# 0xSameer/ast

Hardware: AMD Instinct MI355X
Metric: speech frames/s (train step) (higher is better)
Workload: dtype f32 storage / f32 accumulate; batched GEMMs as bf16x3 splits on the bf16 MFMA pipe (every f32 operand value represented EXACTLY by three bf16 terms, f32 exponent range, six term products, each product exact to 2^-26: >= float32 on any data); the encoder recurrences multiply the same way (resident we

## Files before the change

### ast_amd/csrc/common.h

```cpp
#pragma once
#include <hip/hip_runtime.h>
#include <stdint.h>
#include <stddef.h>
#include <stdio.h>
#include <string.h>
#include "../../include/astk.h"

namespace astk {

void set_error(const char* fmt, ...);

enum ProfCat { PROF_ATTN_FWD = 0, PROF_ATTN_BWD = 1, PROF_GEMM = 2, PROF_CELL = 3, PROF_DEC_FWD = 4, PROF_DEC_BWD = 5, PROF_NCAT = 6 };
bool prof_enabled();
float* prof_tick_buffer(int which);
void prof_start(int cat, hipStream_t s, double work);
void prof_stop(int cat, hipStream_t s);
void prof_add_bytes(int cat, double bytes);
struct ProfScope {
  int cat; hipStream_t s; bool on;
  ProfScope(int c, hipStream_t st, double work = 0.0) : cat(c), s(st), on(prof_enabled()) { if (on) prof_start(cat, s, work); }
  ~ProfScope() { if (on) prof_stop(cat, s); }
};

#define ASTK_CHECK(cond, ...)            \
// ... 28 lines not shown
  } while (0)

#define ASTK_TRY(expr)        \
  do {                        \
    int r_ = (expr);          \
    if (r_ != 0) return r_;   \
  } while (0)

enum PersistBit { PERSIST_ENC_FWD = 1, PERSIST_ENC_BWD = 2, PERSIST_DEC_FWD = 4, PERSIST_DEC_BWD = 8 };
struct AbortCtl {
  unsigned* word;
  unsigned* status;
  unsigned limit;
  unsigned bit;
};
AbortCtl abort_ctl(unsigned* word, unsigned bit);
int device_cu_count();
enum TuneKey {
  TUNE_GEMM_TILE, TUNE_GEMM_T256_ABOVE, TUNE_GEMM_GRID, TUNE_GEMM_HYBRID, TUNE_GEMM_CHUNK, TUNE_GEMM_CHUNK_DIV, TUNE_GEMM_LOG, TUNE_GEMM_TICKET,
  TUNE_GEMM_DETERMINISTIC, TUNE_GEMM_FORWARD_PAIRS,
  TUNE_CONV_DIRECT0, TUNE_CONV_SEQ_FWD, TUNE_CONV_SEQ_BWD, TUNE_CONV_SEQ_STATS_BLOCKS, TUNE_CONV_SEQ_APPLY_BLOCKS,
  TUNE_DEC_PERSIST, TUNE_DEC_B6_SPLIT, TUNE_DEC_B6_FUSED, TUNE_DEC_WIDE,
  TUNE_LSTM_PERSIST, TUNE_LSTM_HOIST, TUNE_LSTM_X3, TUNE_LSTM_X4, TUNE_LSTM_ROWS32, TUNE_LSTM_OVERLAP_CHUNK, TUNE_LSTM_SIDE_FWD, TUNE_LSTM_SIDE_BWD, TUNE_LSTM_DUO_SIDE,
  TUNE_ROW_LONGK, TUNE_PERSIST_SPIN_LIMIT, TUNE_COLREDUCE_BLOCKS,
  TUNE_COUNT
};
double tune(TuneKey k);
inline bool tune_on(TuneKey k) { return tune(k) != 0.0; }
__device__ __forceinline__ bool abort_seen(const AbortCtl& ab) {
  return __hip_atomic_load(ab.word, __ATOMIC_RELAXED, __HIP_MEMORY_SCOPE_AGENT) != 0;
}
__device__ __forceinline__ void abort_raise(const AbortCtl& ab) {
  __hip_atomic_store(ab.word, 1u, __ATOMIC_RELAXED, __HIP_MEMORY_SCOPE_AGENT);
  __hip_atomic_fetch_or(ab.status, ab.bit, __ATOMIC_RELAXED, __HIP_MEMORY_SCOPE_AGENT);
}

constexpr int AMAX_SLOT_WORDS = 16;
constexpr int AMAX_PSLOT_STRIDE = 16;
constexpr int AMAX_PSLOT_WORDS = AMAX_SLOT_WORDS * AMAX_PSLOT_STRIDE;
static inline unsigned long long* amax_pslot_handle(unsigned long long* p) { return p ? (unsigned long long*)((uintptr_t)p | 1u) : nullptr; }
static inline __host__ __device__ unsigned long long* amax_shard(const unsigned long long* handle, int i) {
  unsigned long long* base = (unsigned long long*)((uintptr_t)handle & ~(uintptr_t)1);
  return base + (i & (AMAX_SLOT_WORDS - 1)) * (((uintptr_t)handle & 1u) ? AMAX_PSLOT_STRIDE : 1);
}

typedef float f32x4 __attribute__((ext_vector_type(4)));
// ... 141 lines not shown
  long sA, sB, sC;
  int lowp;
  const unsigned long long* amaxA;
  const unsigned long long* amaxB;
  unsigned spanA, spanB;
  int kt;
  int tiles_mn;
  long iters_total;
  int bm;
  int cs;
  long chunk_iters;
};
static inline GemmArgs gemm_args(int M, int N, int K, MatView A, MatView B, float* C, long ldc,
                                 const float* bias = nullptr, int mode = GEMM_STORE, int ksplit = 1) {
  GemmArgs g;
  memset(&g, 0, sizeof(g));
  g.A = A; g.B = B; g.C = C; g.ldc = ldc; g.bias = bias; g.M = M; g.N = N; g.K = K;
  g.mode = mode; g.ksplit = ksplit; g.batch = 1;
  return g;
}
static inline GemmArgs lowp(GemmArgs g) { g.lowp = 1; return g; }
static inline GemmArgs with_amax_a(GemmArgs g, const unsigned long long* a) { g.amaxA = a; return g; }
static inline GemmArgs with_amax_b(GemmArgs g, const unsigned long long* b) { g.amaxB = b; return g; }
int gemm_launch(int layout, const GemmArgs& g, hipStream_t s);
const unsigned long long* gemm_amax(const float* p, long rows, long ld, int inner, hipStream_t s);
void gemm_amax_reserve(int n, unsigned long long** slots, unsigned* gen, hipStream_t s);
const unsigned long long* gemm_amax_bound(float bound, hipStream_t s);
void gemm_amax_step_boundary(hipStream_t s);
struct AmaxMatrix { const float* p; long rows, ld; int inner; };
void gemm_amax_many(const AmaxMatrix* m, int n, const unsigned long long** out, hipStream_t s);
int low_precision_gemms();
int gemm_precision_mode();
struct PrecScope {
  PrecScope(int precision, int operands);
  ~PrecScope();
  int prev_p, prev_l;
};
struct GemmForwardScope {
  GemmForwardScope();
  ~GemmForwardScope();
  int prev;
};
struct DetScope {
  explicit DetScope(int requested);
  ~DetScope();
  int prev;
};
bool deterministic_mode();
struct GemmWgCap {
  explicit GemmWgCap(int wgs);
  ~GemmWgCap();
  int prev;
};
constexpr int GEMM_GROUP_MAX = 12;
struct GemmGroup {
  int n;
  int unit;
  int dp_waves;
  int dp_kt;
  long rem_start;
  long iters_total;
  long iter_start[GEMM_GROUP_MAX + 1];
  unsigned* tick;
  int tick_base[GEMM_GROUP_MAX];
  GemmArgs g[GEMM_GROUP_MAX];
};
int gemm_launch_group(int layout, const GemmArgs* list, int n, hipStream_t s);

const unsigned* persist_status_word();
int status_snapshot_launch(float* dst, hipStream_t s);

int fill_zero(void* p, size_t bytes, hipStream_t s);
constexpr int FILL_SEG_MAX = 16;
struct FillSegs { int n; void* p[FILL_SEG_MAX]; size_t bytes[FILL_SEG_MAX]; unsigned val[FILL_SEG_MAX]; unsigned own[FILL_SEG_MAX]; const void* src[FILL_SEG_MAX]; };
static inline void fill_seg_add(FillSegs& f, void* p, size_t bytes) {
  if (bytes > 0 && f.n < FILL_SEG_MAX) { f.p[f.n] = p; f.bytes[f.n] = bytes; f.own[f.n] = 0; f.val[f.n] = 0; f.src[f.n] = nullptr; ++f.n; }
}
static inline void fill_seg_add(FillSegs& f, void* p, size_t bytes, unsigned value) {
  if (bytes > 0 && f.n < FILL_SEG_MAX) { f.p[f.n] = p; f.bytes[f.n] = bytes; f.own[f.n] = 1; f.val[f.n] = value; f.src[f.n] = nullptr; ++f.n; }
}
static inline void fill_seg_add_copy(FillSegs& f, void* p, const void* src, size_t bytes) {
  if (bytes > 0 && f.n < FILL_SEG_MAX) { f.p[f.n] = p; f.bytes[f.n] = bytes; f.own[f.n] = 0; f.val[f.n] = 0; f.src[f.n] = src; ++f.n; }
}
int fill_u32_segments(const FillSegs& f, unsigned value, hipStream_t s);
struct CopySegs { int n; void* dst[FILL_SEG_MAX]; const void* src[FILL_SEG_MAX]; size_t bytes[FILL_SEG_MAX]; };
static inline void copy_seg_add(CopySegs& c, void* dst, const void* src, size_t bytes) {
  if (bytes > 0 && c.n < FILL_SEG_MAX) { c.dst[c.n] = dst; c.src[c.n] = src; c.bytes[c.n] = bytes; ++c.n; }
// ... 186 lines not shown
```

### ast_amd/csrc/gemm.hip

```cpp
#include "common.h"
#include <cstdio>
#include <cstdlib>
#include <algorithm>
#include <atomic>
#include <mutex>
#include <vector>
#include <type_traits>

namespace astk {

namespace {

#ifndef ASTK_GEMM_BK
#define ASTK_GEMM_BK 16
#endif
constexpr int BK = ASTK_GEMM_BK;
#ifndef ASTK_GEMM_RING
#define ASTK_GEMM_RING 4
#endif
#ifndef ASTK_GEMM_RING8
#define ASTK_GEMM_RING8 2
#endif
#ifndef ASTK_GEMM_PRIO8
#define ASTK_GEMM_PRIO8 3
// ... 58 lines not shown
}
__device__ __forceinline__ void split2(float x0, float x1, unsigned& hi, unsigned& mid, unsigned& lo) {
  hi = cvt_pk_bf16(x0, x1);
  const float r0 = x0 - __uint_as_float(hi << 16), r1 = x1 - __uint_as_float(hi & 0xffff0000u);
  mid = cvt_pk_bf16(r0, r1);
  const float s0 = r0 - __uint_as_float(mid << 16), s1 = r1 - __uint_as_float(mid & 0xffff0000u);
  lo = cvt_pk_bf16(s0, s1);
}
__device__ __forceinline__ int scale_exp(const unsigned long long* amax) {
  if (amax == nullptr) return 127;
  const int st = ((uintptr_t)amax & 1u) ? AMAX_PSLOT_STRIDE : 1;
  amax = (const unsigned long long*)((uintptr_t)amax & ~(uintptr_t)1);
  unsigned long long w = amax[0];
#pragma unroll
  for (int i = 1; i < 16; ++i) w = max(w, amax[i * st]);
  const int e = (int)(((unsigned)w) >> 23) & 0xff;
  return e == 0 ? 127 : min(max(268 - e, 1), 253);
}
constexpr int sp_hs(int TL) { return TL * 16 + 16; }
constexpr int sp_rs(int TL) { return TL * 2 + 64; }
constexpr int sp_plane(int TL, bool RK) { return RK ? (BK / 8) * sp_hs(TL) : BK * sp_rs(TL); }
constexpr int sp_stage(int TL, bool RK, int prec = PREC_BF16X3) { return prec_planes(prec) * sp_plane(TL, RK); }

template <int TL, bool RK, bool TWOLVL, int PREC = PREC_F32, int RING = 1>
struct Stager {
  static constexpr int LD_KR = ld_kr(TL);
  static constexpr int KQ = BK / 4;
  static constexpr int CQ = TL / 4;
  static constexpr int RP = 256 / CQ;
  static constexpr int NP = RK ? TL * KQ / 256 : BK / RP;
  static_assert(NP >= 1 && (RK || RP * NP == BK), "tile / thread-count mismatch");
  float4 reg[RING][NP];
  unsigned voff[NP];
  int tgrp, trem;
  int tcol;
  int a, b;
  int kcur;
  int lds;
  float scl;

  __device__ __forceinline__ void init(const MatView& v, int row0, int nrows, int kbeg, int kend, int tid) {
    kcur = kbeg;
    if (RK) {
      a = tid % KQ;
      b = tid / KQ;
#pragma unroll
      for (int p = 0; p < NP; ++p) voff[p] = (unsigned)((rowoff(v, min(row0 + NP * b + p, nrows - 1)) + a * 4) * 4);
      lds = NP * b * LD_RK + 2 * a;
    } else {
      a = tid % CQ;
      b = tid / CQ;
      const int m = (TL == 128 && PREC == PREC_F32) ? ((a >> 3) & 1) * 64 + (a >> 4) * 32 + (a & 7) * 4 : 4 * a;
      const int col = min(row0 + m, ((nrows + 3) & ~3) - 4);
#pragma unroll
      for (int p = 0; p < NP; ++p)
        voff[p] = (unsigned)(((long)(b + RP * p) * (TWOLVL ? v.st : v.ld) + col) * 4);
      if (TWOLVL) { tgrp = kbeg / v.tn; trem = kbeg % v.tn; tcol = col; }
      lds = b * LD_KR + 4 * a;
    }
  }
  __device__ __forceinline__ void load(const MatView& v, unsigned span, int kend, const int slot = 0) {
    if (RK || !TWOLVL) {
      const long adv = RK ? (long)kcur : (long)kcur * v.ld;
      const __amdgpu_buffer_rsrc_t r =
          __builtin_amdgcn_make_buffer_rsrc(const_cast<float*>(v.p + adv), 0, (int)(span - (unsigned)(adv * 4)), 0x00020000);
#pragma unroll
      for (int p = 0; p < NP; ++p) {
        const u32x4 u = __builtin_amdgcn_raw_buffer_load_b128(r, (int)voff[p], 0, 0);
        reg[slot][p] = make_float4(__uint_as_float(u.x), __uint_as_float(u.y), __uint_as_float(u.z), __uint_as_float(u.w));
      }
    } else {
      if (trem + BK <= v.tn && kcur + BK <= kend) {
        const __amdgpu_buffer_rsrc_t r =
            __builtin_amdgcn_make_buffer_rsrc(const_cast<float*>(v.p + (long)tgrp * v.sg + (long)trem * v.st), 0, 0x7fffffff, 0x00020000);
#pragma unroll
        for (int p = 0; p < NP; ++p) {
          const u32x4 u = __builtin_amdgcn_raw_buffer_load_b128(r, (int)voff[p], 0, 0);
          reg[slot][p] = make_float4(__uint_as_float(u.x), __uint_as_float(u.y), __uint_as_float(u.z), __uint_as_float(u.w));
        }
      } else {
#pragma unroll
        for (int p = 0; p < NP; ++p) {
          const int kr = min(kcur + b + RP * p, kend - 1);
          reg[slot][p] = *reinterpret_cast<const float4*>(v.p + (long)(kr / v.tn) * v.sg + (long)(kr % v.tn) * v.st + tcol);
        }
      }
      trem += BK;
      while (trem >= v.tn) { trem -= v.tn; ++tgrp; }
    }
    kcur += BK;
  }
  __device__ __forceinline__ void load_pair(const MatView& v, unsigned span, const int slot, bool second) {
    static_assert(RING == 1 || (RING % 2) == 0, "pairs of slots");
    const long adv = (long)kcur;
    const __amdgpu_buffer_rsrc_t r =
        __builtin_amdgcn_make_buffer_rsrc(const_cast<float*>(v.p + adv), 0, (int)(span - (unsigned)(adv * 4)), 0x00020000);
#pragma unroll
    for (int p = 0; p < NP; ++p) {
      const u32x4 u = __builtin_amdgcn_raw_buffer_load_b128(r, (int)voff[p], 0, 0);
      reg[slot][p] = make_float4(__uint_as_float(u.x), __uint_as_float(u.y), __uint_as_float(u.z), __uint_as_float(u.w));
      if (second) {
        const u32x4 w = __builtin_amdgcn_raw_buffer_load_b128(r, (int)voff[p] + BK * 4, 0, 0);
        reg[(slot + 1) % RING][p] = make_float4(__uint_as_float(w.x), __uint_as_float(w.y), __uint_as_float(w.z), __uint_as_float(w.w));
      }
    }
    kcur += 2 * BK;
  }
  __device__ __forceinline__ void store(float* S) const {
    if (RK) {
#pragma unroll
      for (int p = 0; p < NP; ++p) {
        *reinterpret_cast<float2*>(&S[lds + p * LD_RK]) = make_float2(reg[0][p].x, reg[0][p].y);
        *reinterpret_cast<float2*>(&S[lds + p * LD_RK + BK / 2]) = make_float2(reg[0][p].z, reg[0][p].w);
      }
    } else {
#pragma unroll
      for (int p = 0; p < NP; ++p) *reinterpret_cast<float4*>(&S[lds + RP * p * LD_KR]) = reg[0][p];
    }
  }
// ... 48 lines not shown
        if (nv < 3) q[BK / 2] = 0.f;
        if (nv < 4) q[BK / 2 + 1] = 0.f;
      }
    } else if (TWOLVL) {
#pragma unroll
      for (int p = 0; p < NP; ++p)
        if (ktile + b + RP * p >= kend) *reinterpret_cast<float4*>(&S[lds + RP * p * LD_KR]) = make_float4(0.f, 0.f, 0.f, 0.f);
    }
  }
};

#ifndef ASTK_GEMM_TICKET
#ifdef ASTK_TEST_HOOKS
#define ASTK_GEMM_TICKET 1
#else
#define ASTK_GEMM_TICKET 0
#endif
#endif
constexpr int TICK_WAVES = 8;
constexpr unsigned TICK_DONE = 1u << 15;
constexpr int gemm_mw(int TLM) { return TLM == 256 ? 8 : 4; }
constexpr int gemm_threads(int PREC, int TLM = 128) { return PREC != PREC_F32 ? 256 + 64 * gemm_mw(TLM) : 256; }
constexpr int gemm_min_waves(int TL, int PREC, int TLM) { return (PREC != PREC_F32 && TLM == 256) ? 3 : waves_per_simd(TL, PREC); }
template <int TL, bool A_RK, bool B_RK, bool TWOLVL, int PREC, int TLM = TL, bool FIX = false>
__global__ __launch_bounds__(gemm_threads(PREC, TLM), gemm_min_waves(TL, PREC, TLM)) void gemm_f32_kernel(GemmGroup grp) {
  static_assert(!FIX || (PREC == PREC_BF16X3 && TL == 128 && TLM == 128), "the deterministic fix-up is instantiated for the 128 x 128 bf16x3 kernel");
  constexpr int LD_KR = ld_kr(TL);
  constexpr int LDA = A_RK ? LD_RK : LD_KR;
  constexpr int LDB = B_RK ? LD_RK : LD_KR;
  constexpr bool SPLIT = PREC != PREC_F32;
  constexpr int MW = SPLIT ? gemm_mw(TLM) : 4;
  constexpr int WT = TL / 2, WTM = TLM / (MW / 2);
  constexpr int NA = WT / 32;
  constexpr int NAM = WTM / 32;
  constexpr int NPL = prec_planes(PREC);
  static_assert(SPLIT || TLM == TL, "the f32 path runs square tiles");
  constexpr int A_FLOATS = SPLIT ? sp_stage(TLM, A_RK, PREC) / 4 : (A_RK ? TL * LD_RK : BK * LD_KR);
  constexpr int B_FLOATS = SPLIT ? sp_stage(TL, B_RK, PREC) / 4 : (B_RK ? TL * LD_RK : BK * LD_KR);
  constexpr int NST = SPLIT ? 3 : 2;
  __shared__ __attribute__((aligned(16))) float As[NST][A_FLOATS];
  __shared__ __attribute__((aligned(16))) float Bs[NST][B_FLOATS];
  static_assert(BK == 16 || BK == 32, "BK / 2 floats per lane and operand, read as BK / 8 float4");

  const bool producer = SPLIT && threadIdx.x >= 64 * MW;
  const int tid = producer ? threadIdx.x - 64 * MW : threadIdx.x;
  const bool stages = !SPLIT || producer, multiplies = !SPLIT || !producer;
  const int lane = tid & 63, wave = tid >> 6;
// ... 32 lines not shown
      tile = r / g.cs;
      const int kk = (int)(r - tile * g.cs);
      k0 = (int)c * g.cs + kk;
      k1 = (int)min((long)(k0 - kk + g.cs), (long)k0 + (lend - lit));
    } else {
      tile = lit / kt_tile;
      k0 = (int)(lit - tile * kt_tile);
      k1 = (int)min((long)kt_tile, (long)k0 + (lend - lit));
    }
    it += k1 - k0;
    int zb, m0, n0;
    decode_tile(g, tile, TLM, TL, zb, m0, n0);
    const int m0_t = m0, n0_t = n0;
    const int kbeg = k0 * BK;
    const int kend = min(g.K, k1 * BK);
    const bool whole = (k0 == 0) && (k1 == kt_tile);

    MatView A = g.A, B = g.B;
    A.p += (long)zb * g.sA;
    B.p += (long)zb * g.sB;
    float* C = g.C + (long)zb * g.sC;

    constexpr int RING = SPLIT ? (MW == 8 ? ASTK_GEMM_RING8 : ASTK_GEMM_RING) : 1;
    Stager<TLM, A_RK, TWOLVL, PREC, RING> sa;
    Stager<TL, B_RK, TWOLVL, PREC, RING> sb;
    sa.init(A, m0, g.M, kbeg, kend, tid & 255);
    sb.init(B, n0, g.N, kbeg, kend, tid & 255);
    int seA = 127, seB = 127;
    if constexpr (PREC == PREC_F16X2 || PREC == PREC_F16) {
      seA = scale_exp(g.amaxA);
      seB = scale_exp(g.amaxB);
      sa.scl = __uint_as_float((unsigned)seA << 23);
      sb.scl = __uint_as_float((unsigned)seB << 23);
    }

    const int nk = k1 - k0;
    const bool add_bias = g.bias != nullptr && k0 == 0;
    const int mode = !whole || g.mode == GEMM_ACCUM ? GEMM_ATOMIC : g.mode;
    const int tick_idx = (ASTK_GEMM_TICKET && !whole && g.mode == GEMM_STORE && grp.tick != nullptr) ? (grp.tick_base[prob] + (int)tile) * TICK_WAVES : -1;
    const float* const e_bias = add_bias ? g.bias : nullptr;
    const long fix_gs0 = (FIX && !whole) ? grp.iter_start[prob] + tile * kt_tile : -1;
    const int g_mode = g.mode, e_kt = g.kt;
    const int e_M = g.M, e_N = g.N, e_ctn = g.c_tn;
    const long e_ldc = g.ldc, e_csg = g.c_sg, e_cst = g.c_st;
    auto epilogue = [&](f32x16 (&acc)[NAM][NA]) {
      int m0 = m0_t, n0 = n0_t;
      asm volatile("" : "+v"(m0), "+v"(n0));
      if (e_bias) {
#pragma unroll
        for (int j = 0; j < NA; ++j) {
// ... 699 lines not shown
    if (inner <= 0 || nrows <= 0 || J.n >= AMAX_REGIONS) return;
    AmaxRegion& R = J.r[J.n];
    R.p = p; R.nb = nb; R.sb = sb; R.rows = nrows; R.ld = ld; R.inner = inner; R.slot = slot;
    const double bytes = 4.0 * nb * nrows * inner;
    const int blocks = (int)std::min(1024.0, std::max(1.0, bytes / (32.0 * 1024.0)));
    J.blk_start[J.n + 1] = J.blk_start[J.n] + blocks;
    ++J.n;
  };
  const long outer = kr ? K : rows;
  const int inner = kr ? rows : K;
  if (v.tn > 0 || v.rowidx) {
    const long n = span_floats;
    push(v.p, batch, sbatch, n / 1024, 1024, 1024);
    push(v.p + (n / 1024) * 1024, batch, sbatch, 1, 0, (int)(n % 1024));
  } else if (v.ld == inner && batch == 1) {
    const long n = outer * (long)inner;
    push(v.p, 1, 0, n / 1024, 1024, 1024);
    push(v.p + (n / 1024) * 1024, 1, 0, 1, 0, (int)(n % 1024));
  } else {
    push(v.p, batch, sbatch, outer, v.ld, inner);
  }
}

int gemm_launch_group(int layout, const GemmArgs* list, int n, hipStream_t s) {
  ASTK_CHECK(layout == GEMM_NT || layout == GEMM_NN || layout == GEMM_TN, "gemm: bad layout %d", layout);
  ASTK_CHECK(n >= 0 && n <= GEMM_GROUP_MAX, "gemm: group of %d products (max %d)", n, GEMM_GROUP_MAX);
  GemmGroup grp;
  bool twolvl = false, any_store = false;
  long tiles = 0;
  double flops = 0;
  int min_kt = 0x7fffffff;
  const int force_tl = (int)tune(TUNE_GEMM_TILE);
  int prec = default_prec();
  if (low_precision_gemms() != 0 && n > 0) {
    bool all = true;
    for (int i = 0; i < n; ++i) all = all && list[i].lowp != 0;
    if (all) prec = PREC_F16;
  }
  if (prec == PREC_F16X2 && tl_wg_cap > 0) prec = PREC_BF16X3;
  const bool det = tl_det != 0;
  if (det && prec == PREC_F16X2) prec = PREC_BF16X3;
  int TL = 128, TLM = 128;
  for (int pass = 0; pass < 3; ++pass) {
    memset(&grp, 0, sizeof(grp));
    twolvl = any_store = false;
    tiles = 0; flops = 0; min_kt = 0x7fffffff;
    bool tall_ok = true;
    for (int i = 0; i < n; ++i) {
      const GemmArgs& g = list[i];
      if (g.M <= 0 || g.N <= 0 || g.K <= 0 || g.batch <= 0) continue;
      GemmArgs& a = grp.g[grp.n];
      bool tl = false;
      ASTK_TRY(gemm_prepare(layout, g, a, tl, TLM, TL));
      twolvl = twolvl || tl;
      grp.iter_start[grp.n] = grp.iters_total;
      grp.iters_total += a.iters_total;
      tiles += (long)a.tiles_mn * g.batch;
      flops += 2.0 * g.M * g.N * (double)g.K * g.batch;
      any_store = any_store || g.mode == GEMM_STORE;
      min_kt = std::min(min_kt, a.kt);
      tall_ok = tall_ok && cdiv(g.M, 256) * 256 * 10 <= cdiv(g.M, 128) * 128 * 11;
      ++grp.n;
    }
    if (pass > 0) break;
    int max_kt = 0;
    for (int i = 0; i < grp.n; ++i) max_kt = std::max(max_kt, grp.g[i].kt);
    bool small = grp.iters_total < 256L * wgs_per_cu(128) * 10 * (32 / BK) && (tiles < 192 || max_kt <= 12 * (16 / BK > 0 ? 16 / BK : 1));
    if (tl_wg_cap > 0) small = small && 2 * tiles < tl_wg_cap;
    const double big_flops = tune(TUNE_GEMM_T256_ABOVE);
    const bool big = prec == PREC_BF16X3 && BK == 16 && tall_ok && flops >= big_flops && !small;
    int want = force_tl == 64 || force_tl == 128 || force_tl == 256 ? force_tl : (small ? 64 : (big ? 256 : 128));
    if (det && prec == PREC_BF16X3) want = 128;
    if (want == 256 && (prec != PREC_BF16X3 || BK != 16)) want = 128;
    if (want == 64 && prec == PREC_F16) want = 128;
    if (want == 128) break;
    TLM = want;
    TL = want == 256 ? 128 : want;
  }
  if (prec == PREC_F16X2 && flops < g_small_flops.load()) {
    bool given = true;
    for (int i = 0; i < grp.n; ++i) given = given && grp.g[i].amaxA && grp.g[i].amaxB;
    if (!given) prec = PREC_BF16X3;
  }
  const int WGS_PER_CU = wgs_per_cu(TL, prec);
  if (grp.n == 0) return 0;
  for (int i = grp.n; i <= GEMM_GROUP_MAX; ++i) grp.iter_start[i] = grp.iters_total;
  grp.unit = prec != PREC_F32 ? 2 : 1;
  for (int i = 0; i < grp.n; ++i)
    if (grp.g[i].kt & 1) grp.unit = 1;
  if (twolvl) {
    const bool a_kr = layout == GEMM_TN, b_kr = layout != GEMM_NT;
    for (int i = 0; i < grp.n; ++i) {
      GemmArgs& a = grp.g[i];
      if (a_kr && a.A.tn <= 0) { a.A.tn = 0x7fffffff; a.A.sg = 0; a.A.st = a.A.ld; }
      if (b_kr && a.B.tn <= 0) { a.B.tn = 0x7fffffff; a.B.sg = 0; a.B.st = a.B.ld; }
    }
  }
  const int force_g = (int)tune(TUNE_GEMM_GRID);
  const bool forward_rule = tl_forward != 0 || tune(TUNE_GEMM_FORWARD_PAIRS) >= 2;
  long G = tiles;
  bool aligned = true;
  if (grp.iters_total >= 256L * WGS_PER_CU * 10 * (32 / BK)) { G = 256 * WGS_PER_CU; aligned = false; }
  else if (tiles < 160) {
    const long g2 = std::min(256L, grp.iters_total / (4 * (32 / BK)));
    if (g2 > tiles) { G = g2; aligned = false; }
  }
  if (force_g > 0) { G = std::min<long>(force_g, grp.iters_total); aligned = false; }
  if (tl_wg_cap > 0 && G > tl_wg_cap) { G = tl_wg_cap; aligned = false; }
  if (det && prec != PREC_BF16X3) { G = tiles; aligned = true; }
  if (det && !aligned && G > FIX_WGS) G = FIX_WGS;
  if (aligned && grp.n > 1) {
    bool uniform = true;
// ... 22 lines not shown
    }
  }
  if (forward_rule && !aligned && grp.dp_waves == 0 && tune_on(TUNE_GEMM_FORWARD_PAIRS)) {
    int max_kt = 0;
    bool uniform = true;
    for (int i = 0; i < grp.n; ++i) { max_kt = std::max(max_kt, grp.g[i].kt); uniform = uniform && grp.g[i].kt == grp.g[0].kt; }
    const long gmax = std::max(1L, grp.iters_total / std::max(1, max_kt));
    if (G > gmax) G = (uniform && max_kt % (2 * grp.unit) == 0 && G >= 2 * tiles) ? 2 * tiles : gmax;
  }
  const bool chunk_on = tune_on(TUNE_GEMM_CHUNK);
  const int chunk_div = (int)tune(TUNE_GEMM_CHUNK_DIV);
  for (int i = 0; i < grp.n; ++i) { grp.g[i].cs = 0; grp.g[i].chunk_iters = 0; }
  if (chunk_on && !det && grp.n == 1 && !aligned && grp.dp_waves == 0 && grp.g[0].mode != GEMM_STORE && prec != PREC_F32 && tiles * chunk_div <= G && grp.g[0].kt >= 128) {
    GemmArgs& a = grp.g[0];
    const long share = grp.iters_total / G;
    int best = 0;
    for (int c = 2; c <= a.kt; c += 2)
      if (a.kt % c == 0 && c >= share / 2 && c <= share * 2 && (best == 0 || labs(c - share) < labs(best - share))) best = c;
    if (best > 0 && best < a.kt) { a.cs = best; a.chunk_iters = tiles * (long)best; }
  }
  const bool log_shapes = tune_on(TUNE_GEMM_LOG);
  if (log_shapes)
    for (int i = 0; i < grp.n; ++i)
      fprintf(stderr, "astk_gemm layout=%d M=%d N=%d K=%d batch=%d mode=%d twolvl=%d group=%d/%d G=%ld kt=%d tile=%d dp_waves=%d bm=%d cs=%d\n", layout, grp.g[i].M,
              grp.g[i].N, grp.g[i].K, grp.g[i].batch, grp.g[i].mode, (int)twolvl, i, grp.n, G, grp.g[i].kt, TLM * 1000 + TL, grp.dp_waves, grp.g[i].bm, grp.g[i].cs);
  ProfScope prof(PROF_GEMM, s, flops);
  if (prof_enabled()) {
    double bytes = 0;
    for (int i = 0; i < grp.n; ++i) {
      const GemmArgs& a = grp.g[i];
      bytes += 4.0 * a.batch * ((double)a.M * a.K + (double)a.N * a.K + (double)a.M * a.N * (a.mode == GEMM_STORE ? 1 : 2));
    }
    prof_add_bytes(PROF_GEMM, bytes);
  }
  dim3 grid((unsigned)G, 1, 1);
  const bool ticket_on = ASTK_GEMM_TICKET && tune_on(TUNE_GEMM_TICKET);
  grp.tick = nullptr;
  const bool fixup = det && !aligned && prec == PREC_BF16X3 && TL == 128 && TLM == 128;
  bool need_zero = !aligned && any_store && G > 1 && !fixup;
  if (need_zero && ticket_on) {
    long ntiles = 0;
    bool fits = true;
    for (int i = 0; i < grp.n; ++i) {
      grp.tick_base[i] = (int)ntiles;
      ntiles += (grp.iter_start[i + 1] - grp.iter_start[i]) / grp.g[i].kt;
      fits = fits && grp.g[i].kt < (int)TICK_DONE;
    }
    if (fits && ntiles < (1L << 27)) {
// ... 35 lines not shown
    if (log_shapes)
      for (int i = 0; i < J.n; ++i)
        fprintf(stderr, "astk_gemm absmax region %d/%d: %ld x %ld rows (ld %ld) x %d floats = %.1f MB, %d blocks\n", i, J.n, J.r[i].nb, J.r[i].rows, J.r[i].ld,
                J.r[i].inner, 4e-6 * J.r[i].nb * J.r[i].rows * J.r[i].inner, J.blk_start[i + 1] - J.blk_start[i]);
    amax_blocks = J.n > 0 ? J.blk_start[J.n] : 0;
    if (amax_blocks > 0) {
      if (need_zero) hipLaunchKernelGGL(k_absmax_zero, dim3((unsigned)(amax_blocks + (G - 1) * ZERO_PARTS)), dim3(256), 0, s, J, grp, (int)G, TLM, TL, zero_vec ? 1 : 0);
      else hipLaunchKernelGGL(k_absmax, dim3((unsigned)amax_blocks), dim3(256), 0, s, J);
    }
  }
  if (need_zero && amax_blocks == 0) hipLaunchKernelGGL(k_zero_split_tiles, dim3((unsigned)((G - 1) * ZERO_PARTS)), dim3(256), 0, s, grp, (int)G, TLM, TL, zero_vec ? 1 : 0);
#define ASTK_GEMM_LAUNCH(T_, P_, M_)                                                                                              \
  switch (layout) {                                                                                                               \
    case GEMM_NT: hipLaunchKernelGGL((gemm_f32_kernel<T_, true, true, false, P_, M_>), grid, dim3(gemm_threads(P_, M_)), 0, s, grp); break;  \
    case GEMM_NN:                                                                                                                 \
      if (twolvl) hipLaunchKernelGGL((gemm_f32_kernel<T_, true, false, true, P_, M_>), grid, dim3(gemm_threads(P_, M_)), 0, s, grp);  \
      else hipLaunchKernelGGL((gemm_f32_kernel<T_, true, false, false, P_, M_>), grid, dim3(gemm_threads(P_, M_)), 0, s, grp);        \
      break;                                                                                                                      \
    default:                                                                                                                      \
      if (twolvl) hipLaunchKernelGGL((gemm_f32_kernel<T_, false, false, true, P_, M_>), grid, dim3(gemm_threads(P_, M_)), 0, s, grp); \
      else hipLaunchKernelGGL((gemm_f32_kernel<T_, false, false, false, P_, M_>), grid, dim3(gemm_threads(P_, M_)), 0, s, grp);       \
      break;                                                                                                                      \
  }
  if (prec == PREC_F32) {
    if (TL == 64) { ASTK_GEMM_LAUNCH(64, PREC_F32, 64) } else { ASTK_GEMM_LAUNCH(128, PREC_F32, 128) }
  } else if (prec == PREC_F16) { ASTK_GEMM_LAUNCH(128, PREC_F16, 128)
  } else if (prec == PREC_F16X2) {
    if (TL == 64) { ASTK_GEMM_LAUNCH(64, PREC_F16X2, 64) } else { ASTK_GEMM_LAUNCH(128, PREC_F16X2, 128) }
  } else if (TLM == 256) {
    if constexpr (BK == 16) { ASTK_GEMM_LAUNCH(128, PREC_BF16X3, 256) }
  } else if (TL == 64) { ASTK_GEMM_LAUNCH(64, PREC_BF16X3, 64)
  } else if (fixup) {
    switch (layout) {
      case GEMM_NT: hipLaunchKernelGGL((gemm_f32_kernel<128, true, true, false, PREC_BF16X3, 128, true>), grid, dim3(gemm_threads(PREC_BF16X3, 128)), 0, s, grp); break;
      case GEMM_NN:
        if (twolvl) hipLaunchKernelGGL((gemm_f32_kernel<128, true, false, true, PREC_BF16X3, 128, true>), grid, dim3(gemm_threads(PREC_BF16X3, 128)), 0, s, grp);
        else hipLaunchKernelGGL((gemm_f32_kernel<128, true, false, false, PREC_BF16X3, 128, true>), grid, dim3(gemm_threads(PREC_BF16X3, 128)), 0, s, grp);
        break;
      default:
        if (twolvl) hipLaunchKernelGGL((gemm_f32_kernel<128, false, false, true, PREC_BF16X3, 128, true>), grid, dim3(gemm_threads(PREC_BF16X3, 128)), 0, s, grp);
        else hipLaunchKernelGGL((gemm_f32_kernel<128, false, false, false, PREC_BF16X3, 128, true>), grid, dim3(gemm_threads(PREC_BF16X3, 128)), 0, s, grp);
        break;
    }
  } else { ASTK_GEMM_LAUNCH(128, PREC_BF16X3, 128) }
#undef ASTK_GEMM_LAUNCH
  ASTK_LAUNCH_CHECK();
  return 0;
}

int gemm_launch(int layout, const GemmArgs& g, hipStream_t s) { return gemm_launch_group(layout, &g, 1, s); }

void gemm_amax_many(const AmaxMatrix* m, int n, const unsigned long long** out, hipStream_t s) {
  for (int i = 0; i < n; ++i) out[i] = nullptr;
  unsigned long long* ring = amax_ring();
  if (default_prec() != PREC_F16X2 || !ring) return;
  ProfScope prof(PROF_GEMM, s, 0.0);
  AmaxJobs J;
  memset(&J, 0, sizeof(J));
  J.gen = next_amax_gen(s);
  for (int i = 0; i < n; ++i) {
    if (!m[i].p || m[i].rows <= 0 || m[i].inner <= 0) continue;
    if (J.n + 2 > AMAX_REGIONS) {
      hipLaunchKernelGGL(k_absmax, dim3((unsigned)J.blk_start[J.n]), dim3(256), 0, s, J);
      const unsigned gen = J.gen;
      memset(&J, 0, sizeof(J));
      J.gen = gen;
    }
    unsigned long long* slot = ring + AMAX_SLOTS / 2 + (size_t)(g_amax_handle.fetch_add(1) % (AMAX_RING_SLOTS / 2)) * AMAX_SLOT_WORDS;
    amax_add(J, mat(m[i].p, m[i].ld), false, (int)m[i].rows, m[i].inner, 1, 0, 0, slot);
    out[i] = slot;
  }
  if (J.n > 0) hipLaunchKernelGGL(k_absmax, dim3((unsigned)J.blk_start[J.n]), dim3(256), 0, s, J);
}
// ... 82 lines not shown
```

### ast_amd/csrc/lstm.hip

```cpp
#include "common.h"
#include <algorithm>
#include <vector>

namespace astk {

struct PersistCellHost {
  const float *Wl, *Wu, *bias, *zx, *xin, *mask, *WlT, *d_enc, *d_hT, *d_cT;
  float *gates, *C, *HR, *HD, *enc;
  const float* WuT;
  float *PR, *PD;
  const float* PD_up;
  int up_external;
  int reverse_pos, layer;
  unsigned long long* amax;
  float* db;
  long dy_sb, dy_st;
  const unsigned* zx_flags; int zx_s0, zx_cs;
  unsigned* prog; int prog_cs;
  float* db_part;
};
bool lstm_persist_hoisted(int h);
bool lstm_persist_applicable(int T, int B, int h, int nl, int nd);
int lstm_persist_rows(int B, int h, int nl, int nd, bool side);
int lstm_persist_layers_per_launch(int B, int h, int nl, int nd, int rows);
// ... 507 lines not shown
      const int rows_d = lstm_persist_hoisted(h) ? 16 : rows_b;
      j.nby = rows_d == 16 ? (B + 15) / 16 : rows_d == 33 ? 2 * ((B + 31) / 32) : (B + 31) / 32;
      for (int i = 0; i < j.n; ++i) { j.db[i] = cells[i].db; j.part[i] = cells[i].db_part; }
      hipLaunchKernelGGL(k_fold_db, dim3(cdiv(4 * h, 256), j.n), dim3(256), 0, s, j);
      ASTK_LAUNCH_CHECK();
    }
  }
  GemmArgs wg[GEMM_GROUP_MAX];
  int nwg = 0;
  const unsigned long long* ax = (d->x_amax && (((uintptr_t)d->x_amax) & 1u)) ? P.ax : (const unsigned long long*)d->x_amax;
  const unsigned long long* aw0[2] = {nullptr, nullptr};
  {
    AmaxMatrix am[3] = {{ax ? nullptr : x, (long)T * B, (long)P.in, P.in}, {dx ? prm[0].Wu : nullptr, 4L * h, (long)P.in, P.in},
                        {dx && P.nd > 1 ? prm[P.nl].Wu : nullptr, 4L * h, (long)P.in, P.in}};
    const unsigned long long* out[3];
    gemm_amax_many(am, 3, out, s);
    if (!ax) ax = out[0];
    aw0[0] = out[1]; aw0[1] = out[2];
  }
  const unsigned long long* ahb = d->out_bound > 0.f ? gemm_amax_bound(exp2f(ceilf(log2f(d->out_bound))), s) : nullptr;
  const unsigned long long* adz_all[16] = {nullptr};
  if (persist)
    for (int i = 0; i < P.nd * P.nl; ++i) adz_all[i] = dz_amax[i];
  ColsumBatch cb;
  for (int l = P.nl - 1; l >= 0; --l) {
    const bool top = l == P.nl - 1;
    const int in = l == 0 ? P.in : h;
    for (int dd = 0; dd < P.nd && !persist; ++dd)
      ASTK_TRY(transpose_f32(P.WlT[dd][l], 4 * h, prm[dd * P.nl + l].Wl, h, 4 * h, h, s));
    for (int i = T - 1; i >= 0 && !persist; --i) {
      LstmCellBwdArgs cells[2];
      for (int dd = 0; dd < P.nd; ++dd) {
        LstmCellBwdArgs& c = cells[dd];
        memset(&c, 0, sizeof(c));
        c.npairs = 1;
        const bool last = i == T - 1;
        c.p[0].A = last ? nullptr : P.ZG[dd][l] + (size_t)(i + 1) * B * 4 * h;
        c.p[0].lda = 4 * h;
        c.p[0].W = P.WlT[dd][l];
        c.p[0].ldw = 4 * h;
        c.p[0].K = last ? 0 : 4 * h;
        c.B = B; c.h = h;
        c.dh_add = (last && d_hT) ? d_hT + ((size_t)dd * P.nl + l) * bh : nullptr;
        if (top) {
          const int pos = dd == 0 ? i : T - 1 - i;
          c.dy2 = d_enc + (size_t)pos * H + (size_t)dd * h;
// ... 23 lines not shown
        wg[nwg++] = with_amax_b(with_amax_a(gemm_args(4 * h, h, rows - B, mat(dz + (size_t)B * 4 * h, 4 * h), mat(P.HR[dd][l], h), g.dWl, h, nullptr, GEMM_ATOMIC, 1), adz), ahb);
      }
      {
        MatView Xv;
        const float* dzu = dz;
        if (l == 0) {
          Xv = mat(x, in);
          if (dd == 1) {
            hipLaunchKernelGGL(k_gather_rows, dim3(2048), dim3(256), 0, s, P.GATH, dz, rows_inv, rows, h);
            ASTK_LAUNCH_CHECK();
            dzu = P.GATH;
          }
        } else Xv = mat(masks ? P.HD[dd][l - 1] : P.HR[dd][l - 1], h);
        if (l == 0 && (dd == 1 || low_precision_gemms())) {
          ASTK_TRY(gemm_launch(GEMM_TN, with_amax_b(with_amax_a(lowp(gemm_args(4 * h, in, rows, mat(dzu, 4 * h), Xv, g.dWu, in, nullptr, GEMM_ATOMIC, 1)), adz), l == 0 ? ax : nullptr), s));
        } else {
          if (nwg == GEMM_GROUP_MAX) { ASTK_TRY(gemm_launch_group(GEMM_TN, wg, nwg, s)); nwg = 0; }
          wg[nwg++] = with_amax_b(with_amax_a(gemm_args(4 * h, in, rows, mat(dzu, 4 * h), Xv, g.dWu, in, nullptr, GEMM_ATOMIC, 1), adz), l == 0 ? ax : ahb);
        }
      }
      if (!persist) ASTK_TRY(cb.add(g.db, dz, 4 * h, rows, 4 * h, s));
      if (l > 0) {
        if (!persist) ASTK_TRY(gemm_launch(GEMM_NN, with_amax_a(gemm_args(rows, h, 4 * h, mat(dz, 4 * h), mat(p.Wu, h), P.DX[dd], h), adz), s));
      } else if (dx && bside.n == 0) {
        MatView A = dd == 0 ? mat(dz, 4 * h) : mat_idx(dz, 4 * h, rows_inv);
        ASTK_TRY(gemm_launch(GEMM_NN, with_amax_b(with_amax_a(lowp(gemm_args(rows, in, 4 * h, A, mat(p.Wu, in), dx, in, nullptr, dd == 0 ? GEMM_STORE : GEMM_ACCUM)), adz), aw0[dd]), s));
      } else if (dx) {
        if (dd == 0) ASTK_TRY(stream_order((hipStream_t)d->side_stream, s));
        const int i1 = T - bside.n * bside.cs;
        if (i1 > 0) ASTK_TRY(dx_steps(dd, 0, i1, s, adz, aw0[dd]));
      }
    }
  }
  ASTK_TRY(cb.flush(s));
  if (nwg > 0) ASTK_TRY(gemm_launch_group(GEMM_TN, wg, nwg, s));
  if (bside.n > 0) ASTK_TRY(stream_order((hipStream_t)d->side_stream, s));
  return 0;
}

}
```

### ast_amd/csrc/util.hip

```cpp
#include "common.h"
#include <algorithm>
#include <stdarg.h>
#include <vector>
#include <atomic>
#include <mutex>

namespace astk {

static thread_local char g_err[512] = "";

void set_error(const char* fmt, ...) {
  va_list ap;
  va_start(ap, fmt);
  vsnprintf(g_err, sizeof(g_err), fmt, ap);
  va_end(ap);
}
const char* last_error() { return g_err; }

struct ProfState {
  bool on = false;
  std::vector<hipEvent_t> ev[PROF_NCAT];
  double work[PROF_NCAT] = {0, 0, 0, 0, 0, 0};
  double bytes[PROF_NCAT] = {0, 0, 0, 0, 0, 0};
};
// ... 50 lines not shown
    {TUNE_GEMM_CHUNK_DIV, "gemm.chunk_div", 4},
    {TUNE_GEMM_LOG, "gemm.log", 0},
    {TUNE_GEMM_TICKET, "gemm.ticket", 1},
    {TUNE_GEMM_DETERMINISTIC, "gemm.deterministic", 0},
    {TUNE_GEMM_FORWARD_PAIRS, "gemm.forward_pairs", 1},
    {TUNE_CONV_DIRECT0, "conv.direct0", 1},
    {TUNE_CONV_SEQ_FWD, "conv.seq_fwd", 1},
    {TUNE_CONV_SEQ_BWD, "conv.seq_bwd", 1},
    {TUNE_CONV_SEQ_STATS_BLOCKS, "conv.seq_stats_blocks", 1024},
    {TUNE_CONV_SEQ_APPLY_BLOCKS, "conv.seq_apply_blocks", 1024},
    {TUNE_DEC_PERSIST, "dec.persist", 1},
    {TUNE_DEC_B6_SPLIT, "dec.b6_split", 1},
    {TUNE_DEC_B6_FUSED, "dec.b6_fused", 1},
    {TUNE_DEC_WIDE, "dec.wide", 1},
    {TUNE_LSTM_PERSIST, "lstm.persist", 1},
    {TUNE_LSTM_HOIST, "lstm.hoist", 1},
    {TUNE_LSTM_X3, "lstm.x3", 1},
    {TUNE_LSTM_X4, "lstm.x4", 1},
    {TUNE_LSTM_ROWS32, "lstm.rows32", -1},
    {TUNE_LSTM_OVERLAP_CHUNK, "lstm.overlap_chunk", 0},
    {TUNE_LSTM_SIDE_FWD, "lstm.side_fwd", 1},
    {TUNE_LSTM_SIDE_BWD, "lstm.side_bwd", 0},
    {TUNE_LSTM_DUO_SIDE, "lstm.duo_side", 0},
    {TUNE_ROW_LONGK, "row.longk", 2048},
    {TUNE_PERSIST_SPIN_LIMIT, "persist.spin_limit", 0},
    {TUNE_COLREDUCE_BLOCKS, "colreduce.blocks", 256},
};
constexpr bool tune_table_in_order() {
  for (int i = 0; i < TUNE_COUNT; ++i)
    if (g_tune_table[i].key != i) return false;
  return true;
}
static_assert(tune_table_in_order(), "g_tune_table rows must follow enum TuneKey");
static std::atomic<double> g_tune[TUNE_COUNT];
static std::atomic<int> g_tune_init{0};
static void tune_init() {
  if (g_tune_init.load(std::memory_order_acquire)) return;
  static std::mutex mu;
  std::lock_guard<std::mutex> lock(mu);
  if (g_tune_init.load()) return;
  for (int i = 0; i < TUNE_COUNT; ++i) g_tune[i].store(g_tune_table[i].def);
  g_tune_init.store(1, std::memory_order_release);
}
double tune(TuneKey k) { tune_init(); return g_tune[k].load(std::memory_order_relaxed); }
static int tune_find(const char* key) {
  if (!key) return -1;
// ... 752 lines not shown
```

Before: 4.724 million.

## Merge both LSTM direction input-gradient GEMMs into one K-split GEMM

For the bottom bidirectional LSTM layer, the forward and backward input-gradient GEMMs (STORE then ACCUM into dx) are replaced by a single NN GEMM of doubled K. The kernel switches its A/B source pointers at k = 4h, with the backward direction's rows gathered through the inverse row index. This removes one launch and one read-modify-write pass over dx, and gives each tile a longer K loop. The cost is a new kernel instantiation with extra per-load branching and stricter layout and precision preconditions.

```diff
diff --git a/ast_amd/csrc/common.h b/ast_amd/csrc/common.h
--- a/ast_amd/csrc/common.h
+++ b/ast_amd/csrc/common.h
@@ -74,6 +74,7 @@
   TUNE_CONV_DIRECT0, TUNE_CONV_SEQ_FWD, TUNE_CONV_SEQ_BWD, TUNE_CONV_SEQ_STATS_BLOCKS, TUNE_CONV_SEQ_APPLY_BLOCKS,
   TUNE_DEC_PERSIST, TUNE_DEC_B6_SPLIT, TUNE_DEC_B6_FUSED, TUNE_DEC_WIDE,
   TUNE_LSTM_PERSIST, TUNE_LSTM_HOIST, TUNE_LSTM_X3, TUNE_LSTM_X4, TUNE_LSTM_ROWS32, TUNE_LSTM_OVERLAP_CHUNK, TUNE_LSTM_SIDE_FWD, TUNE_LSTM_SIDE_BWD, TUNE_LSTM_DUO_SIDE,
+  TUNE_LSTM_MERGED_DX,
   TUNE_ROW_LONGK, TUNE_PERSIST_SPIN_LIMIT, TUNE_COLREDUCE_BLOCKS,
   TUNE_COUNT
 };
@@ -261,7 +262,11 @@
 static inline GemmArgs lowp(GemmArgs g) { g.lowp = 1; return g; }
 static inline GemmArgs with_amax_a(GemmArgs g, const unsigned long long* a) { g.amaxA = a; return g; }
 static inline GemmArgs with_amax_b(GemmArgs g, const unsigned long long* b) { g.amaxB = b; return g; }
-int gemm_launch(int layout, const GemmArgs& g, hipStream_t s);
+struct GemmKSplit {
+  int k2;
+  MatView A2, B2;
+};
+int gemm_launch(int layout, const GemmArgs& g, hipStream_t s, const GemmKSplit* ks = nullptr);
 const unsigned long long* gemm_amax(const float* p, long rows, long ld, int inner, hipStream_t s);
 void gemm_amax_reserve(int n, unsigned long long** slots, unsigned* gen, hipStream_t s);
 const unsigned long long* gemm_amax_bound(float bound, hipStream_t s);
@@ -302,6 +307,10 @@
   long iter_start[GEMM_GROUP_MAX + 1];
   unsigned* tick;
   int tick_base[GEMM_GROUP_MAX];
+  int k2;
+  MatView A2;
+  const float* B2_p;
+  unsigned spanA2, spanB2;
   GemmArgs g[GEMM_GROUP_MAX];
 };
 int gemm_launch_group(int layout, const GemmArgs* list, int n, hipStream_t s);
diff --git a/ast_amd/csrc/gemm.hip b/ast_amd/csrc/gemm.hip
--- a/ast_amd/csrc/gemm.hip
+++ b/ast_amd/csrc/gemm.hip
@@ -104,7 +104,7 @@
 constexpr int sp_plane(int TL, bool RK) { return RK ? (BK / 8) * sp_hs(TL) : BK * sp_rs(TL); }
 constexpr int sp_stage(int TL, bool RK, int prec = PREC_BF16X3) { return prec_planes(prec) * sp_plane(TL, RK); }
 
-template <int TL, bool RK, bool TWOLVL, int PREC = PREC_F32, int RING = 1>
+template <int TL, bool RK, bool TWOLVL, int PREC = PREC_F32, int RING = 1, bool KS = false>
 struct Stager {
   static constexpr int LD_KR = ld_kr(TL);
   static constexpr int KQ = BK / 4;
@@ -114,6 +114,10 @@
   static_assert(NP >= 1 && (RK || RP * NP == BK), "tile / thread-count mismatch");
   float4 reg[RING][NP];
   unsigned voff[NP];
+  unsigned voff2[KS && RK ? NP : 1];
+  int k2;
+  const float* p2;
+  unsigned span2;
   int tgrp, trem;
   int tcol;
   int a, b;
@@ -121,13 +125,25 @@
   int lds;
   float scl;
 
-  __device__ __forceinline__ void init(const MatView& v, int row0, int nrows, int kbeg, int kend, int tid) {
+  __device__ __forceinline__ void init(const MatView& v, int row0, int nrows, int kbeg, int kend, int tid, int ks = 0, const MatView* v2 = nullptr,
+                                       unsigned sp2 = 0) {
     kcur = kbeg;
+    if constexpr (KS) { k2 = ks; p2 = v2->p; span2 = sp2; }
     if (RK) {
       a = tid % KQ;
       b = tid / KQ;
-#pragma unroll
-      for (int p = 0; p < NP; ++p) voff[p] = (unsigned)((rowoff(v, min(row0 + NP * b + p, nrows - 1)) + a * 4) * 4);
+      if constexpr (KS) {
+        const bool second = kbeg >= k2;
+#pragma unroll
+        for (int p = 0; p < NP; ++p) {
+          const int r = min(row0 + NP * b + p, nrows - 1);
+          voff[p] = (unsigned)(((second ? rowoff(*v2, r) : rowoff(v, r)) + a * 4) * 4);
+          if (k2 < kend) voff2[p] = (unsigned)((rowoff(*v2, r) + a * 4) * 4);
+        }
+      } else {
+#pragma unroll
+        for (int p = 0; p < NP; ++p) voff[p] = (unsigned)((rowoff(v, min(row0 + NP * b + p, nrows - 1)) + a * 4) * 4);
+      }
       lds = NP * b * LD_RK + 2 * a;
     } else {
       a = tid % CQ;
@@ -143,9 +159,12 @@
   }
   __device__ __forceinline__ void load(const MatView& v, unsigned span, int kend, const int slot = 0) {
     if (RK || !TWOLVL) {
-      const long adv = RK ? (long)kcur : (long)kcur * v.ld;
+      cross_k2();
+      const bool src2 = KS && kcur >= k2;
+      const long kk = src2 ? kcur - k2 : kcur;
+      const long adv = RK ? kk : kk * v.ld;
       const __amdgpu_buffer_rsrc_t r =
-          __builtin_amdgcn_make_buffer_rsrc(const_cast<float*>(v.p + adv), 0, (int)(span - (unsigned)(adv * 4)), 0x00020000);
+          __builtin_amdgcn_make_buffer_rsrc(const_cast<float*>((src2 ? p2 : v.p) + adv), 0, (int)((src2 ? span2 : span) - (unsigned)(adv * 4)), 0x00020000);
 #pragma unroll
       for (int p = 0; p < NP; ++p) {
         const u32x4 u = __builtin_amdgcn_raw_buffer_load_b128(r, (int)voff[p], 0, 0);
@@ -172,11 +191,19 @@
     }
     kcur += BK;
   }
+  __device__ __forceinline__ void cross_k2() {
+    if (KS && RK && kcur == k2) {
+#pragma unroll
+      for (int p = 0; p < NP; ++p) voff[p] = voff2[p];
+    }
+  }
   __device__ __forceinline__ void load_pair(const MatView& v, unsigned span, const int slot, bool second) {
     static_assert(RING == 1 || (RING % 2) == 0, "pairs of slots");
-    const long adv = (long)kcur;
+    cross_k2();
+    const bool src2 = KS && kcur >= k2;
+    const long adv = src2 ? (long)(kcur - k2) : (long)kcur;
     const __amdgpu_buffer_rsrc_t r =
-        __builtin_amdgcn_make_buffer_rsrc(const_cast<float*>(v.p + adv), 0, (int)(span - (unsigned)(adv * 4)), 0x00020000);
+        __builtin_amdgcn_make_buffer_rsrc(const_cast<float*>((src2 ? p2 : v.p) + adv), 0, (int)((src2 ? span2 : span) - (unsigned)(adv * 4)), 0x00020000);
 #pragma unroll
     for (int p = 0; p < NP; ++p) {
       const u32x4 u = __builtin_amdgcn_raw_buffer_load_b128(r, (int)voff[p], 0, 0);
@@ -271,7 +298,7 @@
 constexpr int gemm_mw(int TLM) { return TLM == 256 ? 8 : 4; }
 constexpr int gemm_threads(int PREC, int TLM = 128) { return PREC != PREC_F32 ? 256 + 64 * gemm_mw(TLM) : 256; }
 constexpr int gemm_min_waves(int TL, int PREC, int TLM) { return (PREC != PREC_F32 && TLM == 256) ? 3 : waves_per_simd(TL, PREC); }
-template <int TL, bool A_RK, bool B_RK, bool TWOLVL, int PREC, int TLM = TL, bool FIX = false>
+template <int TL, bool A_RK, bool B_RK, bool TWOLVL, int PREC, int TLM = TL, bool FIX = false, bool KS = false>
 __global__ __launch_bounds__(gemm_threads(PREC, TLM), gemm_min_waves(TL, PREC, TLM)) void gemm_f32_kernel(GemmGroup grp) {
   static_assert(!FIX || (PREC == PREC_BF16X3 && TL == 128 && TLM == 128), "the deterministic fix-up is instantiated for the 128 x 128 bf16x3 kernel");
   constexpr int LD_KR = ld_kr(TL);
@@ -350,10 +377,17 @@
     float* C = g.C + (long)zb * g.sC;
 
     constexpr int RING = SPLIT ? (MW == 8 ? ASTK_GEMM_RING8 : ASTK_GEMM_RING) : 1;
-    Stager<TLM, A_RK, TWOLVL, PREC, RING> sa;
-    Stager<TL, B_RK, TWOLVL, PREC, RING> sb;
-    sa.init(A, m0, g.M, kbeg, kend, tid & 255);
-    sb.init(B, n0, g.N, kbeg, kend, tid & 255);
+    Stager<TLM, A_RK, TWOLVL, PREC, RING, KS> sa;
+    Stager<TL, B_RK, TWOLVL, PREC, RING, KS> sb;
+    if constexpr (KS) {
+      MatView B2 = B;
+      B2.p = grp.B2_p;
+      sa.init(A, m0, g.M, kbeg, kend, tid & 255, grp.k2, &grp.A2, grp.spanA2);
+      sb.init(B, n0, g.N, kbeg, kend, tid & 255, grp.k2, &B2, grp.spanB2);
+    } else {
+      sa.init(A, m0, g.M, kbeg, kend, tid & 255);
+      sb.init(B, n0, g.N, kbeg, kend, tid & 255);
+    }
     int seA = 127, seB = 127;
     if constexpr (PREC == PREC_F16X2 || PREC == PREC_F16) {
       seA = scale_exp(g.amaxA);
@@ -1099,7 +1133,7 @@
   }
 }
 
-int gemm_launch_group(int layout, const GemmArgs* list, int n, hipStream_t s) {
+static int gemm_launch_impl(int layout, const GemmArgs* list, int n, hipStream_t s, const GemmKSplit* ks) {
   ASTK_CHECK(layout == GEMM_NT || layout == GEMM_NN || layout == GEMM_TN, "gemm: bad layout %d", layout);
   ASTK_CHECK(n >= 0 && n <= GEMM_GROUP_MAX, "gemm: group of %d products (max %d)", n, GEMM_GROUP_MAX);
   GemmGroup grp;
@@ -1117,6 +1151,7 @@
   if (prec == PREC_F16X2 && tl_wg_cap > 0) prec = PREC_BF16X3;
   const bool det = tl_det != 0;
   if (det && prec == PREC_F16X2) prec = PREC_BF16X3;
+  const bool ks_on = ks && ks->k2 > 0;
   int TL = 128, TLM = 128;
   for (int pass = 0; pass < 3; ++pass) {
     memset(&grp, 0, sizeof(grp));
@@ -1150,6 +1185,7 @@
     if (det && prec == PREC_BF16X3) want = 128;
     if (want == 256 && (prec != PREC_BF16X3 || BK != 16)) want = 128;
     if (want == 64 && prec == PREC_F16) want = 128;
+    if (want == 64 && ks_on) want = 128;
     if (want == 128) break;
     TLM = want;
     TL = want == 256 ? 128 : want;
@@ -1165,6 +1201,29 @@
   grp.unit = prec != PREC_F32 ? 2 : 1;
   for (int i = 0; i < grp.n; ++i)
     if (grp.g[i].kt & 1) grp.unit = 1;
+  grp.k2 = 0x7fffffff;
+  if (ks_on) {
+    const GemmArgs& a = grp.g[0];
+    const MatView& A2 = ks->A2;
+    const MatView& B2 = ks->B2;
+    ASTK_CHECK(layout == GEMM_NN && n == 1 && grp.n == 1 && a.batch == 1 && !twolvl,
+               "gemm: a K-split source needs an NN product of one batch slice, no two-level operand");
+    ASTK_CHECK(prec == PREC_BF16X3 && grp.unit == 2 && (TLM == 256 || TL == 128), "gemm: a K-split source needs the bf16x3 scheme (scheme %d) and paired k-iterations", prec);
+    ASTK_CHECK(ks->k2 % (2 * BK) == 0 && ks->k2 < a.K, "gemm: K-split at k = %d: not a multiple of %d below K = %d", ks->k2, 2 * BK, a.K);
+    ASTK_CHECK(A2.p && B2.p && aligned16(A2.p) && aligned16(B2.p), "gemm: K-split source: null or unaligned operand");
+    ASTK_CHECK((A2.ld % 4) == 0 && (A2.sg % 4) == 0 && (A2.st % 4) == 0 && A2.tn >= 0 && B2.tn == 0 && !B2.rowidx && B2.ld == a.B.ld,
+               "gemm: K-split source: A2 rows must be 16-byte aligned, B2 plain rows of B's leading dimension");
+    const long K2 = a.K - ks->k2;
+    const long spa = A2.rowidx ? (A2.idx_rows > 0 ? A2.idx_rows : (long)a.M) * A2.ld
+                               : (A2.tn > 0 ? (long)((a.M - 1) / A2.tn) * A2.sg + (long)(A2.tn - 1) * A2.st : (long)(a.M - 1) * A2.ld) + ((K2 + 3) & ~3L);
+    const long spb = (K2 - 1) * B2.ld + ((a.N + 3) & ~3L);
+    ASTK_CHECK(spa < (1L << 30) && spb < (1L << 30), "gemm: K-split source: an operand spans more than 4 GiB");
+    grp.k2 = ks->k2;
+    grp.A2 = A2;
+    grp.B2_p = B2.p;
+    grp.spanA2 = (unsigned)(spa * 4);
+    grp.spanB2 = (unsigned)(spb * 4);
+  }
   if (twolvl) {
     const bool a_kr = layout == GEMM_TN, b_kr = layout != GEMM_NT;
     for (int i = 0; i < grp.n; ++i) {
@@ -1233,8 +1292,8 @@
   const bool log_shapes = tune_on(TUNE_GEMM_LOG);
   if (log_shapes)
     for (int i = 0; i < grp.n; ++i)
-      fprintf(stderr, "astk_gemm layout=%d M=%d N=%d K=%d batch=%d mode=%d twolvl=%d group=%d/%d G=%ld kt=%d tile=%d dp_waves=%d bm=%d cs=%d\n", layout, grp.g[i].M,
-              grp.g[i].N, grp.g[i].K, grp.g[i].batch, grp.g[i].mode, (int)twolvl, i, grp.n, G, grp.g[i].kt, TLM * 1000 + TL, grp.dp_waves, grp.g[i].bm, grp.g[i].cs);
+      fprintf(stderr, "astk_gemm layout=%d M=%d N=%d K=%d batch=%d mode=%d twolvl=%d group=%d/%d G=%ld kt=%d tile=%d dp_waves=%d bm=%d cs=%d k2=%d\n", layout, grp.g[i].M,
+              grp.g[i].N, grp.g[i].K, grp.g[i].batch, grp.g[i].mode, (int)twolvl, i, grp.n, G, grp.g[i].kt, TLM * 1000 + TL, grp.dp_waves, grp.g[i].bm, grp.g[i].cs, grp.k2 == 0x7fffffff ? 0 : grp.k2);
   ProfScope prof(PROF_GEMM, s, flops);
   if (prof_enabled()) {
     double bytes = 0;
@@ -1316,7 +1375,12 @@
       else hipLaunchKernelGGL((gemm_f32_kernel<T_, false, false, false, P_, M_>), grid, dim3(gemm_threads(P_, M_)), 0, s, grp);       \
       break;                                                                                                                      \
   }
-  if (prec == PREC_F32) {
+  if (ks_on) {
+    if (TLM == 256) {
+      if constexpr (BK == 16) hipLaunchKernelGGL((gemm_f32_kernel<128, true, false, false, PREC_BF16X3, 256, false, true>), grid, dim3(gemm_threads(PREC_BF16X3, 256)), 0, s, grp);
+    } else if (fixup) hipLaunchKernelGGL((gemm_f32_kernel<128, true, false, false, PREC_BF16X3, 128, true, true>), grid, dim3(gemm_threads(PREC_BF16X3, 128)), 0, s, grp);
+    else hipLaunchKernelGGL((gemm_f32_kernel<128, true, false, false, PREC_BF16X3, 128, false, true>), grid, dim3(gemm_threads(PREC_BF16X3, 128)), 0, s, grp);
+  } else if (prec == PREC_F32) {
     if (TL == 64) { ASTK_GEMM_LAUNCH(64, PREC_F32, 64) } else { ASTK_GEMM_LAUNCH(128, PREC_F32, 128) }
   } else if (prec == PREC_F16) { ASTK_GEMM_LAUNCH(128, PREC_F16, 128)
   } else if (prec == PREC_F16X2) {
@@ -1342,7 +1406,8 @@
   return 0;
 }
 
-int gemm_launch(int layout, const GemmArgs& g, hipStream_t s) { return gemm_launch_group(layout, &g, 1, s); }
+int gemm_launch_group(int layout, const GemmArgs* list, int n, hipStream_t s) { return gemm_launch_impl(layout, list, n, s, nullptr); }
+int gemm_launch(int layout, const GemmArgs& g, hipStream_t s, const GemmKSplit* ks) { return gemm_launch_impl(layout, &g, 1, s, ks); }
 
 void gemm_amax_many(const AmaxMatrix* m, int n, const unsigned long long** out, hipStream_t s) {
   for (int i = 0; i < n; ++i) out[i] = nullptr;
diff --git a/ast_amd/csrc/lstm.hip b/ast_amd/csrc/lstm.hip
--- a/ast_amd/csrc/lstm.hip
+++ b/ast_amd/csrc/lstm.hip
@@ -553,6 +553,7 @@
   const unsigned long long* adz_all[16] = {nullptr};
   if (persist)
     for (int i = 0; i < P.nd * P.nl; ++i) adz_all[i] = dz_amax[i];
+  const bool merged_dx = tune_on(TUNE_LSTM_MERGED_DX) && P.nd == 2 && gemm_precision_mode() == 1 && !low_precision_gemms() && (4 * h) % 32 == 0;
   ColsumBatch cb;
   for (int l = P.nl - 1; l >= 0; --l) {
     const bool top = l == P.nl - 1;
@@ -622,6 +623,11 @@
       if (!persist) ASTK_TRY(cb.add(g.db, dz, 4 * h, rows, 4 * h, s));
       if (l > 0) {
         if (!persist) ASTK_TRY(gemm_launch(GEMM_NN, with_amax_a(gemm_args(rows, h, 4 * h, mat(dz, 4 * h), mat(p.Wu, h), P.DX[dd], h), adz), s));
+      } else if (dx && bside.n == 0 && merged_dx) {
+        if (dd == 1) {
+          const GemmKSplit ks = {4 * h, mat_idx(dz, 4 * h, rows_inv), mat(p.Wu, in)};
+          ASTK_TRY(gemm_launch(GEMM_NN, gemm_args(rows, in, 8 * h, mat(P.ZG[0][0], 4 * h), mat(prm[0].Wu, in), dx, in), s, &ks));
+        }
       } else if (dx && bside.n == 0) {
         MatView A = dd == 0 ? mat(dz, 4 * h) : mat_idx(dz, 4 * h, rows_inv);
         ASTK_TRY(gemm_launch(GEMM_NN, with_amax_b(with_amax_a(lowp(gemm_args(rows, in, 4 * h, A, mat(p.Wu, in), dx, in, nullptr, dd == 0 ? GEMM_STORE : GEMM_ACCUM)), adz), aw0[dd]), s));
diff --git a/ast_amd/csrc/util.hip b/ast_amd/csrc/util.hip
--- a/ast_amd/csrc/util.hip
+++ b/ast_amd/csrc/util.hip
@@ -96,6 +96,7 @@
     {TUNE_LSTM_SIDE_FWD, "lstm.side_fwd", 1},
     {TUNE_LSTM_SIDE_BWD, "lstm.side_bwd", 0},
     {TUNE_LSTM_DUO_SIDE, "lstm.duo_side", 0},
+    {TUNE_LSTM_MERGED_DX, "lstm.merged_dx", 1},
     {TUNE_ROW_LONGK, "row.longk", 2048},
     {TUNE_PERSIST_SPIN_LIMIT, "persist.spin_limit", 0},
     {TUNE_COLREDUCE_BLOCKS, "colreduce.blocks", 256},
```

Result: no change. 4.711 million (median of 2 runs) (-0.3%).
